# anisanazim/Movie-Recommendation-Engine

Measured on AMD Instinct MI355X. Metric: item embeddings/sec + top-K ANN queries/sec, ML-25M d=256, 1/2/4/8 GPU, higher is better.
Workload: dtype f64 cdf / f32 features / fp4 sign planes (exact integer Hamming); 1 GPU; SYN-25M (ML-25M-shaped: U=162541 M=59047 R=25000095), F=128 H=256 d=256, 2 GCN layers, W=100 L=2 T=10, LSH 512-bit, 10000 queries K=11, rng=numpy (the reference's np.random MT19937 stream generated on device: neighbour ids bit-exact with the reference CPU path); global_items=59047, queries=10000, parallelism=item-shard x1

## Files before the change

include/pinsage_hip.h:

```cpp
#ifndef PINSAGE_HIP_H
#define PINSAGE_HIP_H

#include <stddef.h>
#include <stdint.h>

#ifdef __cplusplus
extern "C" {
#endif

#define PS_OK 0
#define PS_EINVAL (-1)
#define PS_ELAUNCH (-2)
#define PS_EWORKSPACE (-3)
#define PS_EUNSUPPORTED (-4)

#define PS_RNG_STREAM 0
#define PS_RNG_PHILOX 1
#define PS_RNG_STREAM_RAW 2

#define PS_RNG_STREAM_WALKS 3

#define PS_WALK_HALF_BUCKETS 0x100

typedef void *ps_stream_t;
// ... 31 lines not shown
                   uint64_t seed, uint32_t call, const uint32_t *nodeinfo, const int32_t *guide,
                   const void *packed, const void *buckets, const void *dest_info,
                   int32_t *ids, int32_t *counts, int32_t *nvalid, ps_stream_t stream);

int ps_walk_sample_layers(const int64_t *rowptr, const int32_t *col, const double *cdf, int64_t V,
                          const int64_t *starts, int64_t B, int W, int L, int T,
                          int rng_mode, const double *uniforms, const int64_t *uoff, int64_t layer_stride,
                          uint64_t seed, uint32_t call, const uint32_t *nodeinfo, const int32_t *guide,
                          const void *packed, const void *buckets, const void *dest_info, int layers,
                          int32_t *ids, int32_t *counts, int32_t *nvalid, ps_stream_t stream);

int ps_walk_paths(const int64_t *rowptr, const int32_t *col, const double *cdf, int64_t V,
                  const int64_t *starts, int64_t B, int L, int rng_mode, const double *uniforms,
                  const int64_t *uoff, uint64_t seed, uint32_t call, int walk_mod,
                  const uint32_t *nodeinfo, const int32_t *guide, int32_t *paths, ps_stream_t stream);

int ps_walk_paths_biased(const int64_t *rowptr, const int32_t *col, const double *wsorted, const double *cdf,
                         const int32_t *nbr_sorted, int64_t V, const int64_t *starts, int64_t B, int L, int rng_mode,
                         const double *uniforms, const int64_t *uoff, uint64_t seed, uint32_t call, int walk_mod,
                         const double *bias, int32_t *paths, ps_stream_t stream);
int ps_paths_topk_max_entries(void);
int ps_paths_topk(const int32_t *paths, int64_t B, int n, int T, int32_t *ids, int32_t *counts, int32_t *nvalid,
                  ps_stream_t stream);

int ps_uniform_offsets(const int64_t *rowptr, int64_t V, const int64_t *starts, int64_t B, int W, int L,
                       int64_t *uoff, int64_t *total, ps_stream_t stream);

int ps_mt19937_chunk_log2(void);
int ps_mt19937_window_shift(void);
int ps_mt19937_raw_stream(const uint32_t *state_in, int pos_in, int64_t n, uint32_t *raw, uint32_t *state_out,
                          int32_t *pos_out, const uint32_t *jump_polys, int jump_levels, const uint32_t *radix_polys,
                          int radix_levels, const uint32_t *window_polys, int n_window, const int64_t *ranges,
                          int n_ranges, void *workspace, size_t workspace_bytes, ps_stream_t stream);
size_t ps_mt19937_workspace_bytes(int64_t skip, int64_t n);
int ps_mt19937_random_sample(const uint32_t *state_in, int pos_in, int64_t skip, int64_t n, double *out,
                             uint32_t *state_out, int32_t *pos_out, const uint32_t *jump_polys, int jump_levels,
                             const uint32_t *radix_polys, int radix_levels, const uint32_t *window_polys, int n_window,
                             void *workspace, size_t workspace_bytes, ps_stream_t stream);

int ps_importance_pool(const float *x, int64_t N, int H, const int32_t *ids, const int32_t *counts,
                       const float *wts, const int32_t *nvalid, int64_t B, int T, int64_t max_idx,
                       int renorm, float *out, ps_stream_t stream);

int ps_attention_weights(const float *u, const float *v, int64_t N, int Hd, const float *w2, const int32_t *ids,
                         const int32_t *nvalid, int64_t B, int T, float *attn, ps_stream_t stream);
int ps_gather_max(const float *x, int64_t N, int H, const int32_t *ids, const int32_t *nvalid, int64_t B, int T, float *out,
                  ps_stream_t stream);

int ps_pool_weights(const int32_t *ids, const int32_t *counts, const float *wts, const int32_t *nvalid, int64_t B, int T,
                    int64_t max_idx, int renorm, int lanes, float *w_eff, ps_stream_t stream);
int ps_gather_bwd_segment(void);
size_t ps_gather_bwd_workspace_bytes(int64_t B, int T, int H);
int ps_gather_bwd(const int64_t *rptr, const int32_t *slots, int64_t N, int T, const float *coef, const int32_t *arg,
                  const float *g, int64_t B, int H, float *gx, void *workspace, size_t workspace_bytes, ps_stream_t stream);
int ps_gather_max_arg(const float *x, int64_t N, int H, const int32_t *ids, const int32_t *nvalid, int64_t B, int T, float *out,
                      int32_t *arg, ps_stream_t stream);
size_t ps_attention_bwd_rows_workspace_bytes(int64_t B, int Hd);
int ps_attention_bwd_rows(const float *x, int64_t N, int H, const float *u, const float *v, int Hd, const float *w2,
                          const int32_t *ids, const int32_t *nvalid, const float *attn, const float *g, int64_t B, int T, float *ds,
                          float *du, float *dw2, void *workspace, size_t workspace_bytes, ps_stream_t stream);
int ps_attention_bwd_cols(const int64_t *rptr, const int32_t *slots, int64_t N, int T, const float *ds, const float *u,
                          const float *v, int Hd, const float *w2, int64_t B, float *dv, void *workspace, size_t workspace_bytes,
                          ps_stream_t stream);

size_t ps_bn_stats_workspace_bytes(int64_t M, int N);
int ps_bn_batch_stats(const float *z, int64_t M, int N, const float *gamma, float eps, float momentum, float *running_mean,
// ... 150 lines not shown
```

movie-recommendation-engine_amd/csrc/mt19937.hip:

```cpp
#include "ps_common.h"

#ifndef PS_MT_DEBUG
#define PS_MT_DEBUG 0
#endif

namespace {

constexpr int MT_N = 624, MT_M = 397;
constexpr int DEG = 19937;
constexpr int CHUNK_LOG2 = 17;
constexpr int64_t CHUNK = (int64_t)1 << CHUNK_LOG2;

struct WinSet { int n; long long first[4]; long long cum[5]; };
struct Wanted { int n; long long lo[4], hi[4]; };
__host__ __device__ __forceinline__ long long win_of(const WinSet &ws, long long q) {
    long long w = ws.first[0] + q;
#pragma unroll
    for (int i = 1; i < 4; ++i)
        if (i < ws.n && q >= ws.cum[i]) w = ws.first[i] + (q - ws.cum[i]);
    return w;
}

__device__ __forceinline__ uint32_t twist(uint32_t u, uint32_t v) {
    const uint32_t y = (u & 0x80000000u) | (v & 0x7fffffffu);
// ... 514 lines not shown
    int pos_out;
    int64_t w_lo, w_hi;
    int64_t c0, c1;
};

Plan make_plan(int pos_in, int64_t skip, int64_t n) {
    Plan p;
    p.wa = 2 * skip;
    p.wb = 2 * (skip + n);
    const int64_t consumed = pos_in + p.wb;
    int64_t q = consumed / MT_N, r = consumed % MT_N;
    if (r == 0 && p.wb > 0) { q -= 1; r = MT_N; }
    p.pos_out = (int)r;
    p.key_w = q * MT_N - pos_in;
    p.w_lo = p.wa;
    if (p.key_w >= 0 && p.key_w < p.w_lo) p.w_lo = p.key_w;
    p.w_hi = p.wb;
    if (p.key_w >= 0 && p.key_w + MT_N > p.w_hi) p.w_hi = p.key_w + MT_N;
    const int64_t first = p.w_lo < 1 ? 1 : p.w_lo, last = p.w_hi - 1;
    p.c0 = (first - 1 + HALF) / CHUNK;
    p.c1 = last >= 1 ? (last - 1 + HALF) / CHUNK : 0;
    if (p.c1 < p.c0) p.c1 = p.c0;
    return p;
}

}

extern "C" int ps_mt19937_chunk_log2(void) { return CHUNK_LOG2; }
extern "C" int ps_mt19937_window_shift(void) { return XB * MT_N; }

static int mt_generate(const uint32_t *state_in, int pos_in, int64_t skip, int64_t n, double *out, uint32_t *raw_out,
                       uint32_t *state_out, int32_t *pos_out, const uint32_t *jump_polys, int jump_levels,
                       const uint32_t *radix_polys, int radix_levels, const uint32_t *window_polys, int n_window,
                       const int64_t *ranges_host, int n_ranges, void *workspace, size_t workspace_bytes, ps_stream_t stream);

extern "C" int ps_mt19937_random_sample(const uint32_t *state_in, int pos_in, int64_t skip, int64_t n, double *out,
                                        uint32_t *state_out, int32_t *pos_out, const uint32_t *jump_polys,
                                        int jump_levels, const uint32_t *radix_polys, int radix_levels,
                                        const uint32_t *window_polys, int n_window, void *workspace,
                                        size_t workspace_bytes, ps_stream_t stream) {
    return mt_generate(state_in, pos_in, skip, n, out, nullptr, state_out, pos_out, jump_polys, jump_levels, radix_polys,
                       radix_levels, window_polys, n_window, nullptr, 0, workspace, workspace_bytes, stream);
}

extern "C" int ps_mt19937_raw_stream(const uint32_t *state_in, int pos_in, int64_t n, uint32_t *raw, uint32_t *state_out,
                                     int32_t *pos_out, const uint32_t *jump_polys, int jump_levels,
                                     const uint32_t *radix_polys, int radix_levels, const uint32_t *window_polys,
                                     int n_window, const int64_t *ranges_host, int n_ranges, void *workspace,
                                     size_t workspace_bytes, ps_stream_t stream) {
    if (!raw || !jump_polys || !workspace || n < (1 << 17) || n_ranges < 0 || (n_ranges > 0 && !ranges_host)) return PS_EINVAL;
    return mt_generate(state_in, pos_in, 0, n, nullptr, raw, state_out, pos_out, jump_polys, jump_levels, radix_polys,
                       radix_levels, window_polys, n_window, ranges_host, n_ranges, workspace, workspace_bytes, stream);
}

extern "C" size_t ps_mt19937_workspace_bytes(int64_t skip, int64_t n) {
    if (n < 0 || skip < 0) return 0;
    const Plan p = make_plan(MT_N, skip, n);
    int64_t K = p.c1 - p.c0 + 3;
    if (K < 128) K = 128;
    const size_t states = ps_align256((size_t)(K + 4) * JP * MT_N * 4);
    const size_t seqs = ps_align256((size_t)(K / 2 + 2) * SEQ_PAD * 4);
    return states + seqs + ps_align256((size_t)(p.w_hi - p.w_lo + 2 * MT_N + CHUNK) * 4) + 4096;
}

static int mt_generate(const uint32_t *state_in, int pos_in, int64_t skip, int64_t n, double *out, uint32_t *raw_out,
                       uint32_t *state_out, int32_t *pos_out, const uint32_t *jump_polys,
                       int jump_levels, const uint32_t *radix_polys, int radix_levels, const uint32_t *window_polys,
                       int n_window, const int64_t *ranges_host, int n_ranges, void *workspace, size_t workspace_bytes,
                       ps_stream_t stream) {
    if (!state_in || !state_out || !pos_out || n < 0 || skip < 0 || pos_in < 0 || pos_in > MT_N) return PS_EINVAL;
    if (n > 0 && !out && !raw_out) return PS_EINVAL;
    hipStream_t st = ps_stream(stream);
    if (n == 0 && skip == 0) {
        if (ps_copy_async(state_out, state_in, MT_N * 4, st) != hipSuccess) return PS_ELAUNCH;
        hipLaunchKernelGGL(mt_set_pos_kernel, dim3(1), dim3(1), 0, st, pos_in, pos_out);
        PS_CHECK_LAUNCH();
        return PS_OK;
    }
    const bool parallel = jump_polys != nullptr && workspace != nullptr && (skip > 0 || n >= (1 << 17));
    if (!parallel) {
        if (skip != 0) return PS_EUNSUPPORTED;
        hipLaunchKernelGGL(mt_words_kernel, dim3(1), dim3(256), 0, st, state_in, pos_in, 2 * n,
                           reinterpret_cast<uint32_t *>(out), state_out, pos_out);
        PS_CHECK_LAUNCH();
        if (n > 0) {
            int64_t grid = ps_cdiv(n, 256);
            if (grid > 8192) grid = 8192;
            hipLaunchKernelGGL(mt_pairs_to_double_kernel, dim3((unsigned)grid), dim3(256), 0, st, out, n);
            PS_CHECK_LAUNCH();
        }
        return PS_OK;
    }
    const Plan p = make_plan(pos_in, skip, n);
    const int64_t K = p.c1 - p.c0 + 1;
    if (workspace_bytes < ps_mt19937_workspace_bytes(skip, n)) return PS_EWORKSPACE;
    if ((p.c1 >> (jump_levels - CHUNK_LOG2)) != 0) return PS_EUNSUPPORTED;
    char *base = ps_ws_base(workspace);
    const size_t WSZ = (size_t)JP * MT_N;
    uint32_t *states = reinterpret_cast<uint32_t *>(base);
    const int64_t Kc = K > 126 ? K : 126;
    uint32_t *tmpA = states + (size_t)(Kc + 1) * WSZ;
    uint32_t *tmpB = tmpA + WSZ;
// ... 161 lines not shown
                return PS_OK;
            };
            int rc = round(1, polyA1, JA, PARTS_A, 0, 32);
            if (rc != PS_OK) return rc;
            rc = round(nsrcB, polyA0, 31, PARTS_B, 32, 1);
            if (rc != PS_OK) return rc;
            plain_states = true;
        }
    }
    if (plain_states) {
    } else if (radix_polys && radix_levels > 0) {
        int lvl = 0;
        for (int64_t have = 1; have < K; have *= 32, ++lvl) {
            if (lvl >= radix_levels) return PS_EUNSUPPORTED;
            const int64_t nsrc = (K - have) < have ? (K - have) : have;
            const int64_t jmax = ((K - 1) / have) < 31 ? ((K - 1) / have) : 31;
            hipLaunchKernelGGL(mt_expand_kernel, dim3((unsigned)nsrc), dim3(256), 0, st, states, JP, (int64_t)WSZ, seqs);
            PS_CHECK_LAUNCH();
            hipLaunchKernelGGL(mt_combine_radix_kernel, dim3((unsigned)(nsrc * JP), (unsigned)jmax), dim3(192), 0, st, seqs,
                               radix_polys + (size_t)lvl * 31 * MT_N, states, have, K);
            PS_CHECK_LAUNCH();
        }
    } else {
        for (int m = 0; ((int64_t)1 << m) < K; ++m) {
            const int64_t have = (int64_t)1 << m;
            const int64_t make = (K - have) < have ? (K - have) : have;
            hipLaunchKernelGGL(mt_expand_kernel, dim3((unsigned)make), dim3(256), 0, st, states, JP, (int64_t)WSZ, seqs);
            PS_CHECK_LAUNCH();
            hipLaunchKernelGGL(mt_combine_kernel, dim3((unsigned)(make * JP)), dim3(192), 0, st, seqs,
                               jump_polys + (size_t)(CHUNK_LOG2 + m) * MT_N, states + (size_t)have * WSZ);
            PS_CHECK_LAUNCH();
        }
    }
    const int64_t key_fold = p.key_w >= 1 ? p.key_w : -(int64_t)4 * MT_N;
    if (ranged)
        hipLaunchKernelGGL(mt_chunk_kernel<true>, dim3((unsigned)Kw, 2), dim3(256), 0, st, plain_states ? plainS : states, plain_states ? 1 : JP,
                           p.c0, ws, wt, p.w_lo, raw, key_fold, state_out, p.pos_out, pos_out, word0);
    else
        hipLaunchKernelGGL(mt_chunk_kernel<false>, dim3((unsigned)Kw, 2), dim3(256), 0, st, plain_states ? plainS : states, plain_states ? 1 : JP,
                           p.c0, ws, wt, p.w_lo, raw, key_fold, state_out, p.pos_out, pos_out, word0);
    PS_CHECK_LAUNCH();
    if (n > 0 && !raw_out) {
        int64_t grid = ps_cdiv(n, 256);
        if (grid > 8192) grid = 8192;
        hipLaunchKernelGGL(mt_raw_to_double_kernel, dim3((unsigned)grid), dim3(256), 0, st, raw, p.w_lo, skip, n, out);
        PS_CHECK_LAUNCH();
    }
    if (p.key_w >= 1) {
    } else if (p.key_w == 0) {
        hipLaunchKernelGGL(mt_final_state_kernel, dim3(1), dim3(640), 0, st, raw, p.w_lo, p.key_w, p.pos_out, state_out, pos_out);
        PS_CHECK_LAUNCH();
    } else {
        if (ps_copy_async(state_out, state_in, MT_N * 4, st) != hipSuccess) return PS_ELAUNCH;
        hipLaunchKernelGGL(mt_set_pos_kernel, dim3(1), dim3(1), 0, st, p.pos_out, pos_out);
        PS_CHECK_LAUNCH();
    }
    return PS_OK;
}
```

movie-recommendation-engine_amd/pinsage_hip/dense.py:

```python
from __future__ import annotations

import os

import torch
import torch.nn.functional as F
from torch.autograd.function import once_differentiable

from . import native as nv


def _rowmajor(w):
    if w.dtype != torch.float32:
        raise TypeError("fp32 expected")
    if w.dim() != 2:
        raise ValueError("2-D matrix expected")
    if w.stride(1) != 1 or w.stride(0) < w.size(1):
        w = w.contiguous()
    return w, w.stride(0) if w.size(0) > 1 else max(w.stride(0), w.size(1))


def _require_cuda(*tensors):
    for t in tensors:
        if t is not None and not t.is_cuda:
            raise nv.NativeError("libpinsage_hip takes device (HBM) tensors; got a CPU tensor (no CPU fallback)")


class StagedWeight:
    __slots__ = ("t", "shape")

    def __init__(self, t):
        self.t = t
        self.shape = t.shape

    def size(self, i):
# ... 757 lines not shown
    key = str(dev)
    if key not in _radix_polys_dev:
        from . import mtjump
        import numpy as np
        cl2 = nv.lib().ps_mt19937_chunk_log2()
        _radix_polys_dev[key] = torch.from_numpy(mtjump.radix_polynomials(cl2).view(np.int32)).to(dev).contiguous()
    return _radix_polys_dev[key]


_window_polys_dev = {}


def _window_polys(dev):
    key = str(dev)
    if key not in _window_polys_dev:
        from . import mtjump
        import numpy as np
        cl2, shift = nv.lib().ps_mt19937_chunk_log2(), nv.lib().ps_mt19937_window_shift()
        _window_polys_dev[key] = torch.from_numpy(mtjump.window_polynomials(cl2, shift=shift).view(np.int32)).to(dev).contiguous()
    return _window_polys_dev[key]


_pending_state = []
_handback_host = {}


def _handback_buffer(dev):
    key = str(dev)
    if key not in _handback_host:
        _handback_host[key] = torch.empty(625, dtype=torch.int32).pin_memory()
    return _handback_host[key]


def finish_rng_state():
    import numpy as np
    while _pending_state:
        name, has_gauss, cached, host, ev = _pending_state.pop()
        ev.synchronize()
        words = host.numpy().view(np.uint32).copy()
        np.random.set_state((name, words[:624], int(words[624]), has_gauss, cached))


def mt19937_random_sample(n, device, skip=0, advance=True, parallel=True, radix=True, raw=False, one_round=True, ranges=None):
    import numpy as np
    name, key, pos, has_gauss, cached = np.random.get_state()
    if name != "MT19937":
        raise RuntimeError("numpy global RNG is not MT19937")
    dev = torch.device(device)
    if os.environ.get("PS_MT_SYNC_UPLOAD") == "1":
        st_in = torch.from_numpy(key.astype(np.uint32).view(np.int32)).to(dev)
    else:
        st_in = torch.from_numpy(key.astype(np.uint32).view(np.int32)).pin_memory().to(dev, non_blocking=True)
    st_out = torch.empty(625, dtype=torch.int32, device=dev)
    pos_out = st_out[624:]
    if raw and (skip != 0 or not parallel or n < (1 << 17)):
        raise ValueError("raw stream: skip = 0, the parallel generator and n >= 2^17 are required")
    n, skip, pos = int(n), int(skip), int(pos)
    out = torch.empty(2 * n + 1248, dtype=torch.int32, device=dev) if raw else torch.empty(n, dtype=torch.float64, device=dev)
    polys = _jump_polys(dev) if parallel else None
    rpolys = _radix_polys(dev) if (parallel and radix) else None
    wpolys = _window_polys(dev) if (parallel and radix and one_round) else None
    ws, wsb = nv.workspace("ps_mt19937_workspace_bytes", dev, skip, n) if parallel else (None, 0)
    if ranges is not None and not raw:
        raise ValueError("ranges: raw stream only")
    rg = np.ascontiguousarray(np.asarray(ranges, dtype=np.int64).reshape(-1, 2)) if ranges is not None and len(ranges) else None
    if rg is not None and rg.shape[0] > 3:
        rg = None
    if rg is not None and os.environ.get("PS_MT_POISON") == "1":
        out.fill_(-1)
    levels, rlevels, nwin = (0 if t is None else t.size(0) for t in (polys, rpolys, wpolys))
    with torch.cuda.device(dev):
        if raw:
            nv.call("ps_mt19937_raw_stream", nv.ptr(st_in), pos, n, nv.ptr(out), nv.ptr(st_out), nv.ptr(pos_out), nv.ptr(polys),
                    levels, nv.ptr(rpolys), rlevels, nv.ptr(wpolys), nwin, rg.ctypes.data if rg is not None else None,
                    rg.shape[0] if rg is not None else 0, nv.ptr(ws), wsb, nv.stream())
        else:
            nv.call("ps_mt19937_random_sample", nv.ptr(st_in), pos, skip, n, nv.ptr(out), nv.ptr(st_out), nv.ptr(pos_out),
                    nv.ptr(polys), levels, nv.ptr(rpolys), rlevels, nv.ptr(wpolys), nwin, nv.ptr(ws), wsb, nv.stream())
    if advance == "defer":
        finish_rng_state()
        host = _handback_buffer(dev)
        with torch.cuda.device(dev):
            host.copy_(st_out, non_blocking=True)
            ev = torch.cuda.Event()
            ev.record()
        _pending_state.append((name, has_gauss, cached, host, ev))
    elif advance:
        words = st_out.cpu().numpy().view(np.uint32)
        np.random.set_state((name, words[:624], int(words[624]), has_gauss, cached))
    return out
```

movie-recommendation-engine_amd/pinsage_hip/native.py:

```python
from __future__ import annotations

import ctypes as C
import os

import torch

_HERE = os.path.dirname(os.path.abspath(__file__))
SO_PATH = os.environ.get("PS_HIP_LIB") or os.path.join(_HERE, "libpinsage_hip.so")
_lib = None

PS_RNG_STREAM = 0
PS_RNG_PHILOX = 1
PS_RNG_STREAM_RAW = 2
PS_RNG_STREAM_WALKS = 3
PS_WALK_HALF_BUCKETS = 0x100
PS_RELU = 1
PS_L2NORM = 2
PS_WPERM = 4
PS_LSH_STAGED = 8
PS_HN_PER_QUERY, PS_HN_EXCLUDE_DIAG = 1, 2
PS_LOSS_SHARED, PS_LOSS_PER_QUERY, PS_LOSS_BATCH_HARD = 0, 1, 2
PS_PPR_NO_SKIP = 1
PS_OK, PS_EINVAL, PS_ELAUNCH, PS_EWORKSPACE, PS_EUNSUPPORTED = 0, -1, -2, -3, -4


class LibraryMissing(RuntimeError):
    pass


class NativeError(RuntimeError):
    pass


_CTYPES = {"p": C.c_void_p, "q": C.c_int64, "i": C.c_int, "z": C.c_size_t, "Q": C.c_uint64, "I": C.c_uint32, "f": C.c_float,
           "s": C.c_char_p}
PROTOTYPES = {
    "ps_abi_version": "i",
    "ps_error_string": "s i",
    "ps_csr_build_workspace_bytes": "z qq",
    "ps_csr_build": "i pppqqppppzp",
    "ps_cdf_build": "i ppqpp",
    "ps_guide_build": "i ppqppp",
    "ps_pack_edges": "i pppqpp",
    "ps_bucket_build": "i ppppqqpp",
    "ps_bucket_build_half": "i ppppqqpp",
    "ps_dest_info_build": "i ppqqpp",
    "ps_graph_stats": "i ppqqpp",
    "ps_walk_sample": "i pppqpqiiiippQIppppppppp",
    "ps_walk_sample_layers": "i pppqpqiiiippqQIpppppipppp",
    "ps_walk_paths": "i pppqpqiippQIipppp",
    "ps_walk_paths_biased": "i pppppqpqiippQIippp",
    "ps_paths_topk_max_entries": "i",
    "ps_paths_topk": "i pqiipppp",
    "ps_uniform_offsets": "i pqpqiippp",
    "ps_mt19937_chunk_log2": "i",
    "ps_mt19937_window_shift": "i",
    "ps_mt19937_raw_stream": "i piqppppipipipipzp",
    "ps_mt19937_workspace_bytes": "z qq",
    "ps_mt19937_random_sample": "i piqqppppipipipzp",
    "ps_importance_pool": "i pqippppqiqipp",
    "ps_attention_weights": "i ppqipppqipp",
    "ps_gather_max": "i pqippqipp",
    "ps_pool_weights": "i ppppqiqiipp",
    "ps_gather_bwd_segment": "i",
    "ps_gather_bwd_workspace_bytes": "z qii",
    "ps_gather_bwd": "i ppqipppqippzp",
    "ps_gather_max_arg": "i pqippqippp",
    "ps_attention_bwd_rows_workspace_bytes": "z qi",
    "ps_attention_bwd_rows": "i pqippipppppqippppzp",
    "ps_attention_bwd_cols": "i ppqipppipqppzp",
    "ps_bn_stats_workspace_bytes": "z qi",
    "ps_bn_batch_stats": "i pqipffppppppzp",
    "ps_bn_apply": "i pqipppipp",
    "ps_bn_bwd_workspace_bytes": "z qi",
    "ps_bn_bwd": "i ppqippppfippppzp",
    "ps_layer_norm": "i pqippfppppp",
    "ps_layer_norm_bwd_workspace_bytes": "z qi",
    "ps_layer_norm_bwd": "i ppqippppppppzp",
    "ps_permute_k": "i pqiipp",
    "ps_linear": "i pqipipipipiipp",
    "ps_linear_wgrad_partition": "q q",
    "ps_linear_wgrad_workspace_bytes": "z qii",
    "ps_linear_wgrad": "i pqipipppzp",
    "ps_linear_epilogue_bwd": "i ppqiipp",
    "ps_gcn_layer_workspace_bytes": "z qi",
    "ps_gcn_layer": "i pqipipipqippppiqipiippzp",
    "ps_gcn_order": "i ppiqiqppp",
    "ps_gcn_layer_ordered": "i pqipipipqippppiqipiippzppp",
    "ps_lsh_stage_bytes": "z ii",
    "ps_lsh_stage": "i piipzp",
# ... 154 lines not shown
```

movie-recommendation-engine_amd/pinsage_hip/sampling.py:

```python
from __future__ import annotations

import math
import os

import numpy as np
import torch

from . import native as nv


class NeighborBatch:

    def __init__(self, ids, counts, nvalid):
        self.ids, self.counts, self.nvalid = ids, counts, nvalid
        self._host = None

    @property
    def B(self):
        return int(self.ids.size(0))

    @property
    def T(self):
        return int(self.ids.size(1))

# ... 74 lines not shown

    def __getitem__(self, i):
        self._fill()
        return super().__getitem__(i)

    def __eq__(self, other):
        self._fill()
        return super().__eq__(other)

    def __repr__(self):
        self._fill()
        return super().__repr__()

    def __bool__(self):
        return self.batch.B > 0

    def __reduce__(self):
        self._fill()
        return (list, (list(super().__iter__()),))


def _nodes_tensor(nodes, device, num_nodes):
    if isinstance(nodes, torch.Tensor) and nodes.is_cuda:
        return nodes.to(device=device, dtype=torch.int64).reshape(-1).contiguous()
    a = nodes.numpy() if isinstance(nodes, torch.Tensor) else np.asarray(nodes)
    a = a.astype(np.int64, copy=False).reshape(-1)
    if a.size and (a.min() < -num_nodes or a.max() >= num_nodes):
        raise IndexError("list index out of range")
    if a.size and a.min() < 0:
        a = np.where(a < 0, a + num_nodes, a)
    return torch.from_numpy(np.ascontiguousarray(a)).to(device)


def draw_numpy_uniforms(n, device, defer_state=False, raw=False, ranges=None):
    if n >= (1 << 17):
        from . import dense
        t = dense.mt19937_random_sample(int(n), device, advance="defer" if defer_state else True, raw=raw, ranges=ranges if raw else None)
        return (t, True) if raw else t
    if raw:
        return draw_numpy_uniforms(n, device, defer_state), False
    u = np.random.random_sample(int(n))
    t = torch.from_numpy(u)
    if n:
        t = t.pin_memory()
    return t.to(device, non_blocking=True)


def sink_walk_offsets(graph, starts, W, L, uniforms):
    dev = graph.device
    B = int(starts.numel())
    walks = starts.repeat_interleave(W).contiguous()
    ok = (starts >= 0) & (starts < graph.V)
    deg = torch.zeros(B, dtype=torch.int64, device=dev)
    deg[ok] = graph.rowptr[starts[ok] + 1] - graph.rowptr[starts[ok]]
    steps = ((deg > 0).to(torch.int64) * L).repeat_interleave(W)
    paths = torch.empty((B * W, L), dtype=torch.int32, device=dev)
    off = torch.zeros(B * W, dtype=torch.int64, device=dev)
    for _ in range(B * W + 2):
        off = (torch.cumsum(steps, 0) - steps).contiguous()
        if B * W == 0:
            break
        nv.call("ps_walk_paths", nv.ptr(graph.rowptr), nv.ptr(graph.col), nv.ptr(graph.cdf), graph.V, nv.ptr(walks), B * W, L,
                nv.PS_RNG_STREAM, nv.ptr(uniforms), nv.ptr(off), 0, 0, 0, nv.ptr(graph.nodeinfo), nv.ptr(graph.guide),
                nv.ptr(paths), nv.stream())
        took = (paths >= 0).sum(dim=1)
        if torch.equal(took, steps):
            return off, int(steps.sum().item())
        steps = took
    return off, int(steps.sum().item())

# ... 109 lines not shown
            woff = None
            if uoff is not None:
                woff = (uoff[:, None] + torch.arange(W, dtype=torch.int64, device=dev)[None, :] * L).reshape(-1).contiguous()
            paths = _biased_paths(graph, starts.repeat_interleave(W).contiguous(), L, mode, uniforms, woff, seed, call, W, p, q)
            return paths_topk(paths.view(B, W * L), T)
        ids = torch.empty((B, T), dtype=torch.int32, device=dev)
        counts = torch.empty((B, T), dtype=torch.int32, device=dev)
        nvalid = torch.empty(B, dtype=torch.int32, device=dev)
        packed = use_guide and use_packed
        nv.call("ps_walk_sample", nv.ptr(graph.rowptr), nv.ptr(graph.col), nv.ptr(graph.cdf), graph.V, nv.ptr(starts), B, W, L, T,
                mode | (graph.walk_flags if (use_guide and use_buckets) else 0), nv.ptr(uniforms), nv.ptr(uoff),
                seed & (2 ** 64 - 1), call, nv.ptr(graph.nodeinfo if use_guide else None), nv.ptr(graph.guide if use_guide else None),
                nv.ptr(graph.packed if packed else None),
                nv.ptr(getattr(graph, "buckets", None) if (use_guide and use_buckets) else None),
                nv.ptr(getattr(graph, "dest_info", None) if (packed and use_dest) else None),
                nv.ptr(ids), nv.ptr(counts), nv.ptr(nvalid), nv.stream())
    return NeighborBatch(ids, counts, nvalid)


_range_nodes_dev = {}


def _range_nodes(start, stop, dev):
    key = (str(dev), int(start), int(stop))
    t = _range_nodes_dev.get(key)
    if t is None:
        if len(_range_nodes_dev) >= 64:
            _range_nodes_dev.clear()
        t = _range_nodes_dev[key] = torch.arange(start, stop, dtype=torch.int64, device=dev)
    return t


def walk_sample_layers(graph, nodes, T, layers, W=100, L=2, rng="numpy", seed=0, call=0, uniforms=None,
                       stream_nodes=None, defer_state=False, p=1.0, q=1.0):
    dev = graph.device
    if is_biased(p, q) or (rng == "numpy" and graph.has_reachable_sink):
        nd = torch.arange(nodes.start, nodes.stop, dtype=torch.int64, device=dev) if isinstance(nodes, range) else nodes
        sn = None
        if stream_nodes is not None:
            a0 = stream_nodes[0]
            sn = (torch.arange(a0.start, a0.stop, dtype=torch.int64, device=dev) if isinstance(a0, range) else a0, stream_nodes[1])
        return [walk_sample(graph, nd, T, W, L, rng=rng, seed=seed, call=call + r, uniforms=None, stream_nodes=sn, p=p, q=q)
                for r in range(layers)]
    as_range = nodes if isinstance(nodes, range) else None
    if as_range is not None:
        if as_range.step != 1 or as_range.start < 0 or as_range.stop > graph.V:
            raise IndexError("list index out of range")
        starts = _range_nodes(as_range.start, as_range.stop, dev)
    else:
        starts = _nodes_tensor(nodes, dev, graph.V)
    B = int(starts.numel())
    ids = torch.empty((layers, B, T), dtype=torch.int32, device=dev)
    counts = torch.empty((layers, B, T), dtype=torch.int32, device=dev)
    nvalid = torch.empty((layers, B), dtype=torch.int32, device=dev)
    stride = 0
    with torch.cuda.device(dev):
        if rng == "numpy":
            src = stream_nodes[0] if stream_nodes is not None else (as_range if as_range is not None else starts)
            lo = stream_nodes[1] if stream_nodes is not None else 0
            key = ("uoff", src.start, src.stop, W * L) if isinstance(src, range) and src.step == 1 else None
            cache = graph.__dict__.setdefault("_stream_offsets", {})
            if key is not None and key in cache:
                uoff_all, stride = cache[key]
            else:
                all_t = (torch.arange(src.start, src.stop, dtype=torch.int64, device=dev)
                         if isinstance(src, range) else _nodes_tensor(src, dev, graph.V))
                total = torch.empty(1, dtype=torch.int64, device=dev)
                uoff_all = torch.empty(all_t.numel(), dtype=torch.int64, device=dev)
                nv.call("ps_uniform_offsets", nv.ptr(graph.rowptr), graph.V, nv.ptr(all_t), all_t.numel(), W, L, nv.ptr(uoff_all),
                        nv.ptr(total), nv.stream())
                stride = int(total.item())
                if key is not None:
                    cache[key] = (uoff_all, stride)
            uoff = uoff_all if stream_nodes is None else uoff_all[lo:lo + B].contiguous()
            mode = nv.PS_RNG_STREAM
            if uniforms is None:
                runs = None
                if stream_nodes is not None and B > 0 and B < uoff_all.numel():
                    rkey = None if key is None else key + ("run", lo, B)
                    if rkey is not None and rkey in cache:
                        u_lo, u_hi = cache[rkey]
                    else:
                        u_lo = int(uoff_all[lo].item())
                        u_hi = int(uoff_all[lo + B].item()) if lo + B < uoff_all.numel() else stride
                        if rkey is not None:
                            cache[rkey] = (u_lo, u_hi)
                    if layers <= 3 and os.environ.get("PS_MT_RANGES", "1") != "0":
                        runs = [(r * stride + u_lo, r * stride + u_hi) for r in range(layers)]
                uniforms, is_raw = draw_numpy_uniforms(layers * stride, dev, defer_state=defer_state, raw=True, ranges=runs)
                mode = nv.PS_RNG_STREAM_RAW if is_raw else nv.PS_RNG_STREAM
        elif rng == "philox":
            uoff, uniforms, mode = None, None, nv.PS_RNG_PHILOX
        else:
            raise ValueError("rng must be 'numpy' or 'philox'")
        for r0 in range(0, layers, 8):
            n = min(8, layers - r0)
            u = uniforms
            if uniforms is not None and r0:
                u = uniforms[2 * r0 * stride:] if mode == nv.PS_RNG_STREAM_RAW else uniforms[r0 * stride:]
            nv.call("ps_walk_sample_layers", nv.ptr(graph.rowptr), nv.ptr(graph.col), nv.ptr(graph.cdf), graph.V, nv.ptr(starts), B,
                    W, L, T, mode | graph.walk_flags, nv.ptr(u), nv.ptr(uoff), stride, seed & (2 ** 64 - 1), call + r0,
                    nv.ptr(graph.nodeinfo), nv.ptr(graph.guide), nv.ptr(graph.packed), nv.ptr(getattr(graph, "buckets", None)),
                    nv.ptr(getattr(graph, "dest_info", None)), n, nv.ptr(ids[r0:r0 + n]), nv.ptr(counts[r0:r0 + n]),
                    nv.ptr(nvalid[r0:r0 + n]), nv.stream())
    return [NeighborBatch(ids[r], counts[r], nvalid[r]) for r in range(layers)]


def walk_paths(graph, starts, L, rng="numpy", seed=0, call=0, walk_mod=0, p=1.0, q=1.0):
    dev = graph.device
    biased = is_biased(p, q)
    if biased:
        check_bias(p, q)
        _no_biased_sinks(graph, rng)
    st = _nodes_tensor(starts, dev, graph.V)
    B = int(st.numel())
    paths = torch.empty((B, L), dtype=torch.int32, device=dev)
    with torch.cuda.device(dev):
        if rng == "numpy" and graph.has_reachable_sink:
            uniforms, uoff = _sink_stream(graph, st, 1, L)
            mode = nv.PS_RNG_STREAM
        elif rng == "numpy":
            uoff = torch.empty(B, dtype=torch.int64, device=dev)
# ... 297 lines not shown
```

movie-recommendation-engine_amd/pinsage_hip/shard.py:

```python
from __future__ import annotations

import os

import torch
import torch.distributed as dist

from . import dense, sampling


def shard_range(M, rank, world):
    chunk = (M + world - 1) // world
    lo = min(rank * chunk, M)
    return lo, min(lo + chunk, M), chunk


def _backend(group):
    return dist.get_backend(group) if dist.is_initialized() else None


class _Gather:

    def __init__(self, out, work=None, dev=None):
        self.out, self.work, self.dev = out, work, dev

# ... 46 lines not shown
            return _Gather(out, dev=t.device)
        out = self._buf("recv", tag, (self.world * chunk,) + rest, t.dtype, src.device)
        work = dist.all_gather_into_tensor(out, src, group=self.group, async_op=True)
        return _Gather(out, work)

    def gather_rows(self, t, chunk, tag="rows"):
        return self.gather_rows_async(t, chunk, tag).wait()


def all_gather_rows_async(t, chunk, group=None):
    c = Comm(group)
    return c.gather_rows_async(t, chunk)


def all_gather_rows(t, chunk, group=None):
    return all_gather_rows_async(t, chunk, group).wait()


def fused_self_update(ops, P, i, H):
    Ws, bs = P[f"convs.{i}.lin_self.weight"], P[f"convs.{i}.lin_self.bias"]
    Wu, bu = P[f"convs.{i}.lin_update.weight"], P[f"convs.{i}.lin_update.bias"]
    Wu1 = Wu[:, :H].contiguous()
    W1 = ops.linear(Wu1, Ws.t().contiguous(), None)
    b1 = ops.linear(bs.reshape(1, -1).contiguous(), Wu1, bu).reshape(-1)
    return W1, b1


def refuse_biased(sampler):
    if sampling.is_biased(getattr(sampler, "p", 1.0), getattr(sampler, "q", 1.0)):
        raise ValueError(f"the sharded pipeline does not sample biased walks (p={sampler.p!r}, q={sampler.q!r}): "
                         "use a sampler with p == q == 1, or the unsharded model")


class HipOps:

    def sample(self, sampler, nodes, T, shard=None):
        refuse_biased(sampler)
        if shard is not None and getattr(sampler, "rng", None) == "numpy":
            M, lo = shard
            all_nodes = torch.arange(M, dtype=torch.int64, device=nodes.device)
            return sampler.sample_batch(nodes, T, stream_nodes=(all_nodes, lo))
        return sampler.sample_batch(nodes, T)

    def sample_layers(self, sampler, lo, hi, T, layers, shard=None):
        refuse_biased(sampler)
        stream = None
        if shard is not None and getattr(sampler, "rng", None) == "numpy":
            stream = (range(shard[0]), shard[1])
        return sampler.sample_batches(range(lo, hi), T, layers, stream_nodes=stream, defer_state=True)

    def finish(self):
        dense.finish_rng_state()

    def pool(self, h_full, batch, max_idx):
        return sampling.importance_pool(h_full, batch, max_idx=max_idx)

    def linear(self, x, W, b, x2=None, W2=None, relu=False, l2norm=False):
        return dense.linear(x, W, b, x2=x2, W2=W2, relu=relu, l2norm=l2norm)

    def gcn_layer(self, x, W, b, h_full, batch, max_idx, W2, order=None):
        return dense.gcn_layer(x, W, b, h_full, batch.ids, batch.counts, batch.nvalid, W2, max_idx=max_idx, order=order)

    def gcn_orders(self, batches, max_idx):
        return dense.gcn_orders([b.ids for b in batches], [b.nvalid for b in batches], max_idx)

    def lsh_encode(self, x, A):
        return dense.lsh_encode(x, A)

    def lsh_encode_planes(self, x, A):
        return dense.lsh_encode(x, A, planes=True)

    def stage_weight(self, W):
        return dense.stage_weight(W)

    def stage_lsh(self, A):
        return dense.stage_lsh(A)

    def lsh_planes(self, codes):
        return dense.lsh_expand(codes)

    def hamming_topk(self, q, codes, k, id_offset, planes=None, out=None):
        return dense.hamming_topk(q, codes, k, id_offset=id_offset, planes=planes, out=out)
# ... 21 lines not shown
        self._nodes = {}
        self.overlap_sampling = False
        self.overlap_input_proj = os.environ.get("PS_OVERLAP_INPUT_PROJ") == "1"
        self.fuse_self = True
        self._streams = {}
        self._fused = {}
        self._staged = {}

    def refresh_weights(self, params=None):
        if params is not None:
            self.P = params
        self._fused.clear()
        self._staged.clear()

    def _fused_layer(self, i, H):
        if i not in self._fused:
            self._fused[i] = fused_self_update(self.ops, self.P, i, H)
        return self._fused[i]

    def _w(self, key, W):
        if not hasattr(self.ops, "stage_weight"):
            return W
        t = self._staged.get(key)
        if t is None:
            t = self._staged[key] = self.ops.stage_weight(W)
        return t

    def _side_stream(self, dev):
        key = str(dev)
        if key not in self._streams:
            self._streams[key] = torch.cuda.Stream(device=dev)
        return self._streams[key]

    def _sample(self, nodes, T, shard):
        try:
            return self.ops.sample(self.sampler, nodes, T, shard)
        except TypeError:
            return self.ops.sample(self.sampler, nodes, T)

    def embed(self, x_local, T, x_full=None):
        try:
            return self._embed(x_local, T, x_full)
        finally:
            if hasattr(self.ops, "finish"):
                self.ops.finish()

    def _embed(self, x_local, T, x_full=None):
        ops, P = self.ops, self.P
        dev = x_local.device
        fused = (not (self.overlap_sampling and x_local.is_cuda)) and hasattr(ops, "sample_layers") \
            and hasattr(self.sampler, "sample_batches")
        nodes = None
        if not fused:
            nodes = self._nodes.get(str(dev))
            if nodes is None:
                nodes = self._nodes[str(dev)] = torch.arange(self.lo, self.hi, dtype=torch.int64, device=dev)
        shard = (self.M, self.lo) if self.world > 1 else None
        side = self._side_stream(dev) if (self.overlap_sampling and x_local.is_cuda) else None
        batches, ready = [], []
        early_h = None
        if (self.overlap_input_proj and fused and x_local.is_cuda and getattr(self.sampler, "rng", None) == "numpy"
                and not (x_full is not None and self.world > 1)):
            main = torch.cuda.current_stream(dev)
            aux = self._side_stream(dev)
            aux.wait_stream(main)
            with torch.cuda.stream(aux):
                early_h = ops.linear(x_local, self._w("in", P["input_proj.weight"]), P["input_proj.bias"], relu=True)
                early_ready = aux.record_event()
            early_h.record_stream(main)
        if fused:
            batches = list(ops.sample_layers(self.sampler, self.lo, self.hi, T, self.num_layers, shard))
        elif side is not None:
            main = torch.cuda.current_stream(dev)
            side.wait_stream(main)
            with torch.cuda.stream(side):
                for _ in range(self.num_layers):
                    b = self._sample(nodes, T, shard)
                    for t in (b.ids, b.counts, b.nvalid):
                        t.record_stream(main)
                    batches.append(b)
                    ready.append(side.record_event())
        else:
            batches.append(self._sample(nodes, T, shard))
        orders = None
        if fused and self.fuse_self and hasattr(ops, "gcn_layer") and hasattr(ops, "gcn_orders"):
            orders = ops.gcn_orders(batches, self.M - 1)
        if early_h is not None:
            torch.cuda.current_stream(dev).wait_event(early_ready)
        if x_full is not None and self.world > 1:
            h_all = ops.linear(x_full, self._w("in", P["input_proj.weight"]), P["input_proj.bias"], relu=True)
            h = h_all[self.lo:self.hi]
            pending = _Gather(h_all)
        else:
            h = early_h if early_h is not None else ops.linear(x_local, self._w("in", P["input_proj.weight"]), P["input_proj.bias"], relu=True)
            pending = self.comm.gather_rows_async(h, self.chunk, "h")
        for i in range(self.num_layers):
            if side is None and not fused and i + 1 < self.num_layers:
                batches.append(self._sample(nodes, T, shard))
            H = h.size(1)
            Wu = P[f"convs.{i}.lin_update.weight"]
            if self.fuse_self:
                W1, b1 = self._fused_layer(i, H)
                a_in = h
            else:
                a_in = ops.linear(h, P[f"convs.{i}.lin_self.weight"], P[f"convs.{i}.lin_self.bias"])
                W1, b1 = Wu[:, :H], P[f"convs.{i}.lin_update.bias"]
            h_full = pending.wait()
            if side is not None:
                torch.cuda.current_stream(dev).wait_event(ready[i])
            if self.fuse_self and hasattr(ops, "gcn_layer"):
                kw = {} if orders is None else {"order": orders[i]}
                h = ops.gcn_layer(a_in, self._w(("l1", i), W1), b1, h_full, batches[i], self.M - 1, self._w(("l2", i), Wu[:, H:]), **kw)
            else:
                h_neigh = ops.pool(h_full, batches[i], self.M - 1)
                h = ops.linear(a_in, self._w(("l1", i), W1), b1, x2=h_neigh, W2=self._w(("l2", i), Wu[:, H:]), relu=True, l2norm=True)
            if i + 1 < self.num_layers:
                pending = self.comm.gather_rows_async(h, self.chunk, "h")
        return ops.linear(h, self._w("out", P["output_proj.weight"]), P["output_proj.bias"], l2norm=True)

    def _staged_A(self, A):
# ... 69 lines not shown
```

movie-recommendation-engine_amd/utils/random_walk.py:

```python
from __future__ import annotations

import numpy as np
import torch

from pinsage_hip.graph import DeviceGraph
from pinsage_hip import sampling


class RandomWalkSampler:
    def __init__(self, edge_index, edge_weights=None, walk_length=2, num_walks=100, p=1.0, q=1.0,
                 *, device=None, rng="numpy", seed=0):
        self.edge_index = edge_index
        self.edge_weights = edge_weights
        self.walk_length = walk_length
        self.num_walks = num_walks
        self.p = p
        self.q = q
        self._check_bias()
        self.rng = rng
        self.seed = int(seed)
        self._calls = 0
        self._adj_list = None
        self._prepare_adjacency_list(device)

# ... 2 lines not shown

    def _check_bias(self):
        if sampling.is_biased(self.p, self.q):
            sampling.check_bias(self.p, self.q)

    @classmethod
    def from_graph(cls, graph, walk_length=2, num_walks=100, rng="numpy", seed=0, p=1.0, q=1.0):
        self = cls.__new__(cls)
        self.edge_index = self.edge_weights = None
        self.walk_length, self.num_walks, self.p, self.q = walk_length, num_walks, p, q
        self._check_bias()
        self.rng, self.seed, self._calls, self._adj_list = rng, int(seed), 0, None
        self.graph = graph
        return self

    @property
    def adj_list(self):
        if self._adj_list is None:
            g = self.graph
            rowptr = g.rowptr.cpu().numpy()
            col = g.col.cpu().numpy()
            w = g.wsorted.cpu().numpy()
            self._adj_list = [list(zip(col[rowptr[v]:rowptr[v + 1]].tolist(), w[rowptr[v]:rowptr[v + 1]].tolist()))
                              for v in range(g.V)]
        return self._adj_list

    def sample_batch(self, nodes, num_neighbors=10, uniforms=None, stream_nodes=None):
        call = self._calls
        self._calls += 1
        return sampling.walk_sample(self.graph, nodes, int(num_neighbors), W=self.num_walks, L=self.walk_length,
                                    rng=self.rng, seed=self.seed, call=call, uniforms=uniforms,
                                    stream_nodes=stream_nodes if self.rng == "numpy" else None, p=self.p, q=self.q)

    def sample_batches(self, nodes, num_neighbors=10, layers=2, stream_nodes=None, defer_state=False):
        call = self._calls
        self._calls += layers
        return sampling.walk_sample_layers(self.graph, nodes, int(num_neighbors), int(layers), W=self.num_walks,
                                           L=self.walk_length, rng=self.rng, seed=self.seed, call=call,
                                           stream_nodes=stream_nodes if self.rng == "numpy" else None,
                                           defer_state=defer_state, p=self.p, q=self.q)

    def single_walks(self, start_nodes):
        call = self._calls
        self._calls += 1
        return sampling.walk_paths(self.graph, start_nodes, self.walk_length, rng=self.rng, seed=self.seed, call=call,
                                   p=self.p, q=self.q)

    def _single_walk(self, start_node):
        path = self.single_walks([int(start_node)])[0].tolist()
        walk = [start_node]
        for n in path:
            if n < 0:
                break
            walk.append(np.int64(n))
        return walk

    def sample_neighbors(self, node_idx, num_neighbors=10):
        nb, wt = self.sample_batch([int(node_idx)], num_neighbors).to_lists()
        return nb[0], wt[0]

    def batch_sample_neighbors(self, nodes, num_neighbors=10):
        if isinstance(nodes, torch.Tensor):
            nodes = nodes.tolist()
        batch = self.sample_batch(nodes, num_neighbors)
        return sampling.LazyNeighborList(batch, "ids"), sampling.LazyNeighborList(batch, "weights")

    ppr_method = "device"

    def ppr_batch(self, nodes, num_neighbors=10, alpha=0.15, num_iterations=10, *, max_target=None):
        from pinsage_hip import ppr
        nodes = nodes.tolist() if isinstance(nodes, torch.Tensor) else list(nodes)
        return ppr.ppr_topk(self.graph, nodes, int(num_neighbors), alpha, num_iterations, max_target=max_target)

# ... 82 lines not shown
```

Measured before the change: 48.03 million items/s.

## Overlap input projection with MT19937 chunk kernel via windows-done event hook

Adds a hooked MT19937 raw-stream entry point that records an event once the window/jump phase finishes. The input projection is launched on an auxiliary stream after that event, so it overlaps the chunk-generation and walk kernels rather than the earlier phase. The RNG state upload and handback also now use persistent pinned buffers in place when the state is deferred, which drops per-call device allocations and copies. This adds callback plumbing and cross-stream ordering that has to be gotten right.

Measured after the change: 48.38 million items/s, median of 6. No clear change (+0.7%).

```diff
diff --git a/include/pinsage_hip.h b/include/pinsage_hip.h
--- a/include/pinsage_hip.h
+++ b/include/pinsage_hip.h
@@ -87,6 +87,11 @@
                           int32_t *pos_out, const uint32_t *jump_polys, int jump_levels, const uint32_t *radix_polys,
                           int radix_levels, const uint32_t *window_polys, int n_window, const int64_t *ranges,
                           int n_ranges, void *workspace, size_t workspace_bytes, ps_stream_t stream);
+int ps_mt19937_raw_stream_hooked(const uint32_t *state_in, int pos_in, int64_t n, uint32_t *raw, uint32_t *state_out,
+                                 int32_t *pos_out, const uint32_t *jump_polys, int jump_levels, const uint32_t *radix_polys,
+                                 int radix_levels, const uint32_t *window_polys, int n_window, const int64_t *ranges,
+                                 int n_ranges, void *workspace, size_t workspace_bytes, void *windows_done,
+                                 ps_stream_t stream);
 size_t ps_mt19937_workspace_bytes(int64_t skip, int64_t n);
 int ps_mt19937_random_sample(const uint32_t *state_in, int pos_in, int64_t skip, int64_t n, double *out,
                              uint32_t *state_out, int32_t *pos_out, const uint32_t *jump_polys, int jump_levels,
diff --git a/movie-recommendation-engine_amd/csrc/mt19937.hip b/movie-recommendation-engine_amd/csrc/mt19937.hip
--- a/movie-recommendation-engine_amd/csrc/mt19937.hip
+++ b/movie-recommendation-engine_amd/csrc/mt19937.hip
@@ -570,7 +570,8 @@
 static int mt_generate(const uint32_t *state_in, int pos_in, int64_t skip, int64_t n, double *out, uint32_t *raw_out,
                        uint32_t *state_out, int32_t *pos_out, const uint32_t *jump_polys, int jump_levels,
                        const uint32_t *radix_polys, int radix_levels, const uint32_t *window_polys, int n_window,
-                       const int64_t *ranges_host, int n_ranges, void *workspace, size_t workspace_bytes, ps_stream_t stream);
+                       const int64_t *ranges_host, int n_ranges, void *workspace, size_t workspace_bytes, hipEvent_t windows_done,
+                       ps_stream_t stream);
 
 extern "C" int ps_mt19937_random_sample(const uint32_t *state_in, int pos_in, int64_t skip, int64_t n, double *out,
                                         uint32_t *state_out, int32_t *pos_out, const uint32_t *jump_polys,
@@ -578,7 +579,7 @@
                                         const uint32_t *window_polys, int n_window, void *workspace,
                                         size_t workspace_bytes, ps_stream_t stream) {
     return mt_generate(state_in, pos_in, skip, n, out, nullptr, state_out, pos_out, jump_polys, jump_levels, radix_polys,
-                       radix_levels, window_polys, n_window, nullptr, 0, workspace, workspace_bytes, stream);
+                       radix_levels, window_polys, n_window, nullptr, 0, workspace, workspace_bytes, nullptr, stream);
 }
 
 extern "C" int ps_mt19937_raw_stream(const uint32_t *state_in, int pos_in, int64_t n, uint32_t *raw, uint32_t *state_out,
@@ -588,7 +589,18 @@
                                      size_t workspace_bytes, ps_stream_t stream) {
     if (!raw || !jump_polys || !workspace || n < (1 << 17) || n_ranges < 0 || (n_ranges > 0 && !ranges_host)) return PS_EINVAL;
     return mt_generate(state_in, pos_in, 0, n, nullptr, raw, state_out, pos_out, jump_polys, jump_levels, radix_polys,
-                       radix_levels, window_polys, n_window, ranges_host, n_ranges, workspace, workspace_bytes, stream);
+                       radix_levels, window_polys, n_window, ranges_host, n_ranges, workspace, workspace_bytes, nullptr, stream);
+}
+
+extern "C" int ps_mt19937_raw_stream_hooked(const uint32_t *state_in, int pos_in, int64_t n, uint32_t *raw, uint32_t *state_out,
+                                            int32_t *pos_out, const uint32_t *jump_polys, int jump_levels,
+                                            const uint32_t *radix_polys, int radix_levels, const uint32_t *window_polys,
+                                            int n_window, const int64_t *ranges_host, int n_ranges, void *workspace,
+                                            size_t workspace_bytes, void *windows_done, ps_stream_t stream) {
+    if (!raw || !jump_polys || !workspace || n < (1 << 17) || n_ranges < 0 || (n_ranges > 0 && !ranges_host)) return PS_EINVAL;
+    return mt_generate(state_in, pos_in, 0, n, nullptr, raw, state_out, pos_out, jump_polys, jump_levels, radix_polys,
+                       radix_levels, window_polys, n_window, ranges_host, n_ranges, workspace, workspace_bytes,
+                       static_cast<hipEvent_t>(windows_done), stream);
 }
 
 extern "C" size_t ps_mt19937_workspace_bytes(int64_t skip, int64_t n) {
@@ -605,7 +617,7 @@
                        uint32_t *state_out, int32_t *pos_out, const uint32_t *jump_polys,
                        int jump_levels, const uint32_t *radix_polys, int radix_levels, const uint32_t *window_polys,
                        int n_window, const int64_t *ranges_host, int n_ranges, void *workspace, size_t workspace_bytes,
-                       ps_stream_t stream) {
+                       hipEvent_t windows_done, ps_stream_t stream) {
     if (!state_in || !state_out || !pos_out || n < 0 || skip < 0 || pos_in < 0 || pos_in > MT_N) return PS_EINVAL;
     if (n > 0 && !out && !raw_out) return PS_EINVAL;
     hipStream_t st = ps_stream(stream);
@@ -833,6 +845,7 @@
             PS_CHECK_LAUNCH();
         }
     }
+    if (windows_done && hipEventRecord(windows_done, st) != hipSuccess) return PS_ELAUNCH;
     const int64_t key_fold = p.key_w >= 1 ? p.key_w : -(int64_t)4 * MT_N;
     if (ranged)
         hipLaunchKernelGGL(mt_chunk_kernel<true>, dim3((unsigned)Kw, 2), dim3(256), 0, st, plain_states ? plainS : states, plain_states ? 1 : JP,
diff --git a/movie-recommendation-engine_amd/pinsage_hip/dense.py b/movie-recommendation-engine_amd/pinsage_hip/dense.py
--- a/movie-recommendation-engine_amd/pinsage_hip/dense.py
+++ b/movie-recommendation-engine_amd/pinsage_hip/dense.py
@@ -1,5 +1,6 @@
 from __future__ import annotations
 
+import ctypes as C
 import os
 
 import torch
@@ -823,6 +824,26 @@
     return _handback_host[key]
 
 
+_upload_host = {}
+_hook_events = {}
+
+
+def _upload_buffer(dev):
+    key = str(dev)
+    if key not in _upload_host:
+        _upload_host[key] = torch.empty(624, dtype=torch.int32).pin_memory()
+    return _upload_host[key]
+
+
+def _hook_event(dev):
+    key = str(dev)
+    if key not in _hook_events:
+        ev = torch.cuda.Event()
+        ev.record(torch.cuda.current_stream(dev))
+        _hook_events[key] = ev
+    return _hook_events[key]
+
+
 def finish_rng_state():
     import numpy as np
     while _pending_state:
@@ -832,20 +853,31 @@
         np.random.set_state((name, words[:624], int(words[624]), has_gauss, cached))
 
 
-def mt19937_random_sample(n, device, skip=0, advance=True, parallel=True, radix=True, raw=False, one_round=True, ranges=None):
+def mt19937_random_sample(n, device, skip=0, advance=True, parallel=True, radix=True, raw=False, one_round=True, ranges=None,
+                          on_windows=None):
     import numpy as np
+    if raw and (skip != 0 or not parallel or n < (1 << 17)):
+        raise ValueError("raw stream: skip = 0, the parallel generator and n >= 2^17 are required")
+    if on_windows is not None and not raw:
+        raise ValueError("on_windows: raw stream only")
+    dev = torch.device(device)
+    in_place = raw and advance == "defer" and os.environ.get("PS_MT_STATE_COPIES") != "1"
+    if in_place:
+        finish_rng_state()
     name, key, pos, has_gauss, cached = np.random.get_state()
     if name != "MT19937":
         raise RuntimeError("numpy global RNG is not MT19937")
-    dev = torch.device(device)
-    if os.environ.get("PS_MT_SYNC_UPLOAD") == "1":
-        st_in = torch.from_numpy(key.astype(np.uint32).view(np.int32)).to(dev)
+    if in_place:
+        up, host = _upload_buffer(dev), _handback_buffer(dev)
+        up.numpy().view(np.uint32)[:] = key
+        p_in, p_out, p_pos = (C.c_void_p(a) for a in (up.data_ptr(), host.data_ptr(), host.data_ptr() + 624 * 4))
     else:
-        st_in = torch.from_numpy(key.astype(np.uint32).view(np.int32)).pin_memory().to(dev, non_blocking=True)
-    st_out = torch.empty(625, dtype=torch.int32, device=dev)
-    pos_out = st_out[624:]
-    if raw and (skip != 0 or not parallel or n < (1 << 17)):
-        raise ValueError("raw stream: skip = 0, the parallel generator and n >= 2^17 are required")
+        if os.environ.get("PS_MT_SYNC_UPLOAD") == "1":
+            st_in = torch.from_numpy(key.astype(np.uint32).view(np.int32)).to(dev)
+        else:
+            st_in = torch.from_numpy(key.astype(np.uint32).view(np.int32)).pin_memory().to(dev, non_blocking=True)
+        st_out = torch.empty(625, dtype=torch.int32, device=dev)
+        p_in, p_out, p_pos = nv.ptr(st_in), nv.ptr(st_out), nv.ptr(st_out[624:])
     n, skip, pos = int(n), int(skip), int(pos)
     out = torch.empty(2 * n + 1248, dtype=torch.int32, device=dev) if raw else torch.empty(n, dtype=torch.float64, device=dev)
     polys = _jump_polys(dev) if parallel else None
@@ -861,14 +893,24 @@
         out.fill_(-1)
     levels, rlevels, nwin = (0 if t is None else t.size(0) for t in (polys, rpolys, wpolys))
     with torch.cuda.device(dev):
-        if raw:
-            nv.call("ps_mt19937_raw_stream", nv.ptr(st_in), pos, n, nv.ptr(out), nv.ptr(st_out), nv.ptr(pos_out), nv.ptr(polys),
+        if raw and on_windows is not None:
+            hook = _hook_event(dev)
+            nv.call("ps_mt19937_raw_stream_hooked", p_in, pos, n, nv.ptr(out), p_out, p_pos, nv.ptr(polys),
+                    levels, nv.ptr(rpolys), rlevels, nv.ptr(wpolys), nwin, rg.ctypes.data if rg is not None else None,
+                    rg.shape[0] if rg is not None else 0, nv.ptr(ws), wsb, C.c_void_p(hook.cuda_event), nv.stream())
+        elif raw:
+            nv.call("ps_mt19937_raw_stream", p_in, pos, n, nv.ptr(out), p_out, p_pos, nv.ptr(polys),
                     levels, nv.ptr(rpolys), rlevels, nv.ptr(wpolys), nwin, rg.ctypes.data if rg is not None else None,
                     rg.shape[0] if rg is not None else 0, nv.ptr(ws), wsb, nv.stream())
         else:
-            nv.call("ps_mt19937_random_sample", nv.ptr(st_in), pos, skip, n, nv.ptr(out), nv.ptr(st_out), nv.ptr(pos_out),
+            nv.call("ps_mt19937_random_sample", p_in, pos, skip, n, nv.ptr(out), p_out, p_pos,
                     nv.ptr(polys), levels, nv.ptr(rpolys), rlevels, nv.ptr(wpolys), nwin, nv.ptr(ws), wsb, nv.stream())
-    if advance == "defer":
+    if in_place:
+        with torch.cuda.device(dev):
+            ev = torch.cuda.Event()
+            ev.record()
+        _pending_state.append((name, has_gauss, cached, host, ev))
+    elif advance == "defer":
         finish_rng_state()
         host = _handback_buffer(dev)
         with torch.cuda.device(dev):
@@ -879,4 +921,6 @@
     elif advance:
         words = st_out.cpu().numpy().view(np.uint32)
         np.random.set_state((name, words[:624], int(words[624]), has_gauss, cached))
+    if on_windows is not None:
+        on_windows(hook)
     return out
diff --git a/movie-recommendation-engine_amd/pinsage_hip/native.py b/movie-recommendation-engine_amd/pinsage_hip/native.py
--- a/movie-recommendation-engine_amd/pinsage_hip/native.py
+++ b/movie-recommendation-engine_amd/pinsage_hip/native.py
@@ -56,6 +56,7 @@
     "ps_mt19937_chunk_log2": "i",
     "ps_mt19937_window_shift": "i",
     "ps_mt19937_raw_stream": "i piqppppipipipipzp",
+    "ps_mt19937_raw_stream_hooked": "i piqppppipipipipzpp",
     "ps_mt19937_workspace_bytes": "z qq",
     "ps_mt19937_random_sample": "i piqqppppipipipzp",
     "ps_importance_pool": "i pqippppqiqipp",
diff --git a/movie-recommendation-engine_amd/pinsage_hip/sampling.py b/movie-recommendation-engine_amd/pinsage_hip/sampling.py
--- a/movie-recommendation-engine_amd/pinsage_hip/sampling.py
+++ b/movie-recommendation-engine_amd/pinsage_hip/sampling.py
@@ -130,10 +130,11 @@
     return torch.from_numpy(np.ascontiguousarray(a)).to(device)
 
 
-def draw_numpy_uniforms(n, device, defer_state=False, raw=False, ranges=None):
+def draw_numpy_uniforms(n, device, defer_state=False, raw=False, ranges=None, on_windows=None):
     if n >= (1 << 17):
         from . import dense
-        t = dense.mt19937_random_sample(int(n), device, advance="defer" if defer_state else True, raw=raw, ranges=ranges if raw else None)
+        t = dense.mt19937_random_sample(int(n), device, advance="defer" if defer_state else True, raw=raw, ranges=ranges if raw else None,
+                                        on_windows=on_windows if raw else None)
         return (t, True) if raw else t
     if raw:
         return draw_numpy_uniforms(n, device, defer_state), False
@@ -309,7 +310,7 @@
 
 
 def walk_sample_layers(graph, nodes, T, layers, W=100, L=2, rng="numpy", seed=0, call=0, uniforms=None,
-                       stream_nodes=None, defer_state=False, p=1.0, q=1.0):
+                       stream_nodes=None, defer_state=False, p=1.0, q=1.0, on_windows=None):
     dev = graph.device
     if is_biased(p, q) or (rng == "numpy" and graph.has_reachable_sink):
         nd = torch.arange(nodes.start, nodes.stop, dtype=torch.int64, device=dev) if isinstance(nodes, range) else nodes
@@ -364,7 +365,8 @@
                             cache[rkey] = (u_lo, u_hi)
                     if layers <= 3 and os.environ.get("PS_MT_RANGES", "1") != "0":
                         runs = [(r * stride + u_lo, r * stride + u_hi) for r in range(layers)]
-                uniforms, is_raw = draw_numpy_uniforms(layers * stride, dev, defer_state=defer_state, raw=True, ranges=runs)
+                uniforms, is_raw = draw_numpy_uniforms(layers * stride, dev, defer_state=defer_state, raw=True, ranges=runs,
+                                                               on_windows=on_windows)
                 mode = nv.PS_RNG_STREAM_RAW if is_raw else nv.PS_RNG_STREAM
         elif rng == "philox":
             uoff, uniforms, mode = None, None, nv.PS_RNG_PHILOX
diff --git a/movie-recommendation-engine_amd/pinsage_hip/shard.py b/movie-recommendation-engine_amd/pinsage_hip/shard.py
--- a/movie-recommendation-engine_amd/pinsage_hip/shard.py
+++ b/movie-recommendation-engine_amd/pinsage_hip/shard.py
@@ -102,7 +102,14 @@
                          "use a sampler with p == q == 1, or the unsharded model")
 
 
+def input_proj_overlaps(enabled, fused, on_gpu, rng, has_hook, world, standin, replicated, capturing):
+    if not (enabled and fused and on_gpu and has_hook) or rng != "numpy" or capturing:
+        return False
+    return world == 1 or (standin and not replicated)
+
+
 class HipOps:
+    window_hook = True
 
     def sample(self, sampler, nodes, T, shard=None):
         refuse_biased(sampler)
@@ -112,12 +119,14 @@
             return sampler.sample_batch(nodes, T, stream_nodes=(all_nodes, lo))
         return sampler.sample_batch(nodes, T)
 
-    def sample_layers(self, sampler, lo, hi, T, layers, shard=None):
+    def sample_layers(self, sampler, lo, hi, T, layers, shard=None, on_windows=None):
         refuse_biased(sampler)
         stream = None
         if shard is not None and getattr(sampler, "rng", None) == "numpy":
             stream = (range(shard[0]), shard[1])
-        return sampler.sample_batches(range(lo, hi), T, layers, stream_nodes=stream, defer_state=True)
+        if on_windows is None:
+            return sampler.sample_batches(range(lo, hi), T, layers, stream_nodes=stream, defer_state=True)
+        return sampler.sample_batches(range(lo, hi), T, layers, stream_nodes=stream, defer_state=True, on_windows=on_windows)
 
     def finish(self):
         dense.finish_rng_state()
@@ -205,6 +214,12 @@
             self._streams[key] = torch.cuda.Stream(device=dev)
         return self._streams[key]
 
+    def _overlaps_input_proj(self, fused, x_local, x_full):
+        on_gpu = bool(x_local.is_cuda)
+        return input_proj_overlaps(self.overlap_input_proj, fused, on_gpu, getattr(self.sampler, "rng", None),
+                                   bool(getattr(self.ops, "window_hook", False)), self.world, self.comm.standin is not None,
+                                   x_full is not None, on_gpu and torch.cuda.is_current_stream_capturing())
+
     def _sample(self, nodes, T, shard):
         try:
             return self.ops.sample(self.sampler, nodes, T, shard)
@@ -231,17 +246,20 @@
         shard = (self.M, self.lo) if self.world > 1 else None
         side = self._side_stream(dev) if (self.overlap_sampling and x_local.is_cuda) else None
         batches, ready = [], []
-        early_h = None
-        if (self.overlap_input_proj and fused and x_local.is_cuda and getattr(self.sampler, "rng", None) == "numpy"
-                and not (x_full is not None and self.world > 1)):
+        early = []
+        if self._overlaps_input_proj(fused, x_local, x_full):
             main = torch.cuda.current_stream(dev)
             aux = self._side_stream(dev)
-            aux.wait_stream(main)
-            with torch.cuda.stream(aux):
-                early_h = ops.linear(x_local, self._w("in", P["input_proj.weight"]), P["input_proj.bias"], relu=True)
-                early_ready = aux.record_event()
-            early_h.record_stream(main)
-        if fused:
+            W_in = self._w("in", P["input_proj.weight"])
+
+            def on_windows(windows_done):
+                aux.wait_event(windows_done)
+                with torch.cuda.stream(aux):
+                    h0 = ops.linear(x_local, W_in, P["input_proj.bias"], relu=True)
+                    early.append((h0, aux.record_event()))
+                h0.record_stream(main)
+            batches = list(ops.sample_layers(self.sampler, self.lo, self.hi, T, self.num_layers, shard, on_windows=on_windows))
+        elif fused:
             batches = list(ops.sample_layers(self.sampler, self.lo, self.hi, T, self.num_layers, shard))
         elif side is not None:
             main = torch.cuda.current_stream(dev)
@@ -258,7 +276,9 @@
         orders = None
         if fused and self.fuse_self and hasattr(ops, "gcn_layer") and hasattr(ops, "gcn_orders"):
             orders = ops.gcn_orders(batches, self.M - 1)
-        if early_h is not None:
+        early_h = None
+        if early:
+            early_h, early_ready = early[0]
             torch.cuda.current_stream(dev).wait_event(early_ready)
         if x_full is not None and self.world > 1:
             h_all = ops.linear(x_full, self._w("in", P["input_proj.weight"]), P["input_proj.bias"], relu=True)
diff --git a/movie-recommendation-engine_amd/utils/random_walk.py b/movie-recommendation-engine_amd/utils/random_walk.py
--- a/movie-recommendation-engine_amd/utils/random_walk.py
+++ b/movie-recommendation-engine_amd/utils/random_walk.py
@@ -58,13 +58,14 @@
                                     rng=self.rng, seed=self.seed, call=call, uniforms=uniforms,
                                     stream_nodes=stream_nodes if self.rng == "numpy" else None, p=self.p, q=self.q)
 
-    def sample_batches(self, nodes, num_neighbors=10, layers=2, stream_nodes=None, defer_state=False):
+    def sample_batches(self, nodes, num_neighbors=10, layers=2, stream_nodes=None, defer_state=False, on_windows=None):
         call = self._calls
         self._calls += layers
         return sampling.walk_sample_layers(self.graph, nodes, int(num_neighbors), int(layers), W=self.num_walks,
                                            L=self.walk_length, rng=self.rng, seed=self.seed, call=call,
                                            stream_nodes=stream_nodes if self.rng == "numpy" else None,
-                                           defer_state=defer_state, p=self.p, q=self.q)
+                                           defer_state=defer_state, p=self.p, q=self.q,
+                                           on_windows=on_windows if self.rng == "numpy" else None)
 
     def single_walks(self, start_nodes):
         call = self._calls
```
